# PacificBiosciences/ccs

Measured on AMD Instinct MI355X. Metric: ZMWs/sec (HiFi reads/sec), 10-pass x 10 kb synthetic, higher is better.
Workload: dtype f32

## Files before the change

ccs_amd/csrc/ccsx_kernels.hip:

```cpp
#include <hip/hip_runtime.h>
#include <stdint.h>
#include <cstdio>
#include <cstdlib>

#include "ccsx.h"
#include "ccsx_kernels.h"
#include "wave_ops.h"

#define LANDED(x) asm volatile("" : "+v"(x))

#if (defined(CCSX_EXP_NO_FILL) || defined(CCSX_EXP_NO_SCORE) || defined(CCSX_EXP_ONE_ROUND) || defined(CCSX_EXP_ALL_VALID) || defined(CCSX_EXP_CHEAP_VALIDITY) || \
     defined(CCSX_EXP_NO_ROWS) || defined(CCSX_EXP_NO_SCORE_LOG) || defined(CCSX_EXP_SKIP_ROUND2_SCORE) || defined(CCSX_EXP_NO_QV_EXP) || defined(CCSX_EXP_REPEAT) || defined(CCSX_EXP_NO_BANDMASK) || \
     defined(CCSX_EXP_HOT_PROLOGUE) || defined(CCSX_EXIT_AFTER_PROLOGUE)) && !defined(CCSX_EXPERIMENT)
#error "CCSX_EXP_* / CCSX_EXIT_AFTER_PROLOGUE switches produce wrong results: build them with -DCCSX_EXPERIMENT (never ship such a library)"
#endif
#define CCSX_STR2(x) #x
#define CCSX_STR(x) CCSX_STR2(x)
int ccsx_kernel_is_experiment()
{
#ifdef CCSX_EXPERIMENT
    return 1;
#else
    return 0;
#endif
// ... 1676 lines not shown
                    er = (kq >= 2) ? OMR[(size_t)kq * 64 + (er - loR[kq])].x : 0;
                    ent[nneed - kq] = I - er;
                }
                for (int kq = k1 + 1; kq < k2; ++kq) ent[kq] = -(1 << 20) - 64 * kq;
                dm[0] = 0u;
                for (int kq = 1; kq < nneed; ++kq) dm[kq] = 0x7fffffffu;
                P.avalid[r] = 1; P.ascore[r] = wF + wR;
            }
            continue;
        }
        if (lane == 0) {
            int32_t *ent = P.ent + P.ent_off[r];
            uint32_t *dm = P.dmask + P.ent_off[r];
            const int2 *OMF = (const int2 *)OsF, *OMR = (const int2 *)OsR;
            int e = ks ? ebF[ks] : 0;
            ent[ks] = e;
            for (int k2 = ks; k2 >= 2; --k2) { e = OMF[(size_t)k2 * 64 + (e - loF[k2])].x; ent[k2 - 1] = e; }
            ent[0] = 0;
            const int ksr = nneed - 1 - ks;
            int er = ksr ? ebR[ksr] : 0;
            for (int kq = ksr; kq >= 1; --kq) {
                er = (kq >= 2) ? OMR[(size_t)kq * 64 + (er - loR[kq])].x : 0;
                ent[nneed - kq] = I - er;
            }
            dm[0] = 0u;
            for (int k2 = 1; k2 < nneed; ++k2) dm[k2] = 0x7fffffffu;
            P.avalid[r] = 1; P.ascore[r] = wbest;
        }
      }
    }
}

__global__ void k_post(KParams P, int pass)
{
    int z = blockIdx.x * blockDim.x + threadIdx.x;
    if (z >= P.n_zmw) return;
    const int zr = P.zref[z];
    if (pass && !(zr & ZREF_PASSBIT(pass))) return;
    const bool may_retry = !P.opts.no_fallback_draft && pass < 2;
    const int retry = pass == 0 ? ZREF_RETRY : ((zr & 255) | ZREF_RETRY2);
    if (P.zstat[z] != CCSX_SUCCESS) {
        P.np[z] = 0; P.out_fn[z] = 0; P.out_rn[z] = 0;
        if (may_retry && P.zstat[z] == CCSX_DRAFT_FAILURE) P.zref[z] = retry;
        return;
    }
    int r0 = P.read_off[z], nr = P.nfull[z], np = 0, rn = 0;
    const int f0 = P.flags[r0 + (zr & 255)];
    for (int r = 0; r < nr; ++r) {
        const int v = P.avalid[r0 + r];
        np += v;
        if (v && ((P.flags[r0 + r] ^ f0) & 1)) ++rn;
    }
    P.np[z] = np; P.out_fn[z] = np - rn; P.out_rn[z] = rn;
    if (2 * np <= nr) {
        if (may_retry) P.zref[z] = retry;
        else { P.zstat[z] = CCSX_TOO_MANY_UNUSABLE; P.nwin[z] = 0; }
    }
}

__global__ __launch_bounds__(1024) void k_wmap(KParams P)
{
    __shared__ int sTot[16], sCarry;
    const int tid = threadIdx.x, lane = tid & 63, wv = tid >> 6;
    if (tid == 0) sCarry = 0;
    __syncthreads();
    for (int z0 = 0; z0 < P.n_zmw; z0 += 1024) {
        const int z = z0 + tid;
        const int v = z < P.n_zmw ? P.nwin[z] : 0;
        const int incl = wave_scan_add_i32(v);
        if (lane == 63) sTot[wv] = incl;
        __syncthreads();
        int base = sCarry;
        for (int q = 0; q < wv; ++q) base += sTot[q];
        if (z < P.n_zmw) P.wstart[z] = base + incl - v;
        __syncthreads();
        if (tid == 1023) sCarry = base + incl;
        __syncthreads();
    }
    if (tid == 0) P.wstart[P.n_zmw] = sCarry;
}
__global__ __launch_bounds__(256) void k_wmap_fill(KParams P)
{
    const int z = blockIdx.x * 4 + (threadIdx.x >> 6), lane = threadIdx.x & 63;
    if (z >= P.n_zmw) return;
    const int a = P.wstart[z], nw = P.nwin[z];
    for (int w = lane; w < nw; w += LANES) P.wslot_zmw[a + w] = z;
}

#ifndef PW_THREADS
#define PW_THREADS 256
#endif
#ifndef PW_MINWAVES
#define PW_MINWAVES 4
#endif
#define PW_WAVES (PW_THREADS / 64)
#ifndef PW_CHUNK_READS
#define PW_CHUNK_READS 8
#endif
#ifndef PW_MAXREADS
#define PW_MAXREADS 32
#endif
#ifndef PW_LDS_BYTES
#define PW_LDS_BYTES 40960
#endif
#ifndef CTXS
#define CTXS 17
#endif
#define FILL16_MAXBW 24
#define TC_LO 56
#define TC_HI 38
#define TC_ROW 32
#define TC_STRAND ((CCSX_NOBS + 1) * TC_ROW)
#define DLC_S (33 + TC_LO)
#define DLC_TOTAL (TC_LO + DLC_S + 33 + TC_HI)
#define TAB_TAIL (2 * TC_HI - 48)
#define OBS_TC(o) ((o) * (TC_ROW * 8))
#define OBS_CODE(o) ((o) * (CTXS * 8))

struct LaneMut {
    int c, q, kA, kB, isdel, fin;
    int qoff;
    float dlA, dlL;
};

__device__ __forceinline__ LaneMut lane_mut(int type, int c, int x, const uint8_t *t, int J, int lf, const float *sDL)
{
    LaneMut L;
    const int tm1 = t[c > 0 ? c - 1 : 0];
    const int nidx = (type == 2) ? c : c + 1;
    const int tn = t[nidx < 31 ? nidx : 31];
    const int fin = (type == 2) ? (c == J) : (c + 1 == J);
    const int nx = fin ? 0 : tn;
    int pA = (c > 0) ? tm1 : lf;
    const int xA = (type == 1) ? nx : x;
    if (pA > 3) pA = (xA + 2) & 3;
    const int kA = pA * 4 + xA, kB = (type == 1) ? kA : xA * 4 + nx;
    const int q = (type == 2) ? c + 1 : c + 2;
    L.c = c; L.q = q > J ? J : q; L.isdel = (type == 1); L.fin = fin; L.qoff = (type == 2) ? 0 : 1;
    L.dlA = sDL[kA]; L.dlL = sDL[kB];
    L.kA = (type == 1 && fin) ? (CTXS - 1) : kA;
    L.kB = fin ? (CTXS - 1) : kB;
    return L;
}

typedef const float __attribute__((address_space(3))) *lds_cf;
typedef const char __attribute__((address_space(3))) *lds_cc;

typedef const uint8_t __attribute__((address_space(3))) *lds_cu8;
struct ScoreChain {
    float ap, bp, acc, b, bq;
    float2 pA, pB;
    lds_cf g, be;
    lds_cu8 op;
    int dg;
};

__device__ __forceinline__ float lanes_or_zero(unsigned long long m, float v)
{
    float r;
    asm("v_cndmask_b32_e64 %0, 0, %1, %2" : "=v"(r) : "v"(v), "s"(m));
    return r;
}

__device__ __forceinline__ void score_step(ScoreChain &s, const LaneMut &L, lds_cc tA, lds_cc tB, int pitch, unsigned lim)
{
    typedef const unsigned long long __attribute__((address_space(3))) *lds_cu64;
#ifndef CCSX_EXP_NO_BANDMASK
    const unsigned long long on = __builtin_amdgcn_uicmp((unsigned)s.dg, lim, 37 );
    const float gmm = lanes_or_zero(on, *s.g);
    const float bqn = lanes_or_zero(on, *s.be);
#else
    const float gmm = *s.g, bqn = *s.be;
#endif
    const int o256 = __mul24((int)*s.op, CTXS * 8);
    const unsigned long long va = *(lds_cu64)(tA + o256), vb = *(lds_cu64)(tB + o256);
    const float2 nA = make_float2(__uint_as_float((unsigned)va), __uint_as_float((unsigned)(va >> 32)));
    const float2 nB = make_float2(__uint_as_float((unsigned)vb), __uint_as_float((unsigned)(vb >> 32)));
    s.g += pitch; s.be += pitch; s.op += 1; s.dg -= 1;
    const float insA = s.pA.y, meA = s.pA.x, insB = s.pB.y;
    const float a = __builtin_fmaf(s.ap, insA, gmm);
    float b;
    if (L.isdel) b = a;
    else b = __builtin_fmaf(s.bp, insB, __builtin_fmaf(a, L.dlA, s.ap * meA));
    s.acc = __builtin_fmaf(b, __builtin_fmaf(L.dlL, s.bq, nB.x * bqn), s.acc);
    s.ap = a; s.bp = b; s.b = b; s.pA = nA; s.pB = nB; s.bq = bqn;
}

__device__ __forceinline__ int band_row0(int c, int I, int J2, float invJ2, int J, int Wr, int nrows)
{
    const int num = __mul24(2 * c, I) + J;
    int q = (int)((float)num * invJ2);
    const int r = num - __mul24(q, J2);
    q += (r >= J2 ? 1 : 0) - (r < 0 ? 1 : 0);
    int i0 = q - Wr;
    i0 = i0 < 0 ? 0 : i0;
    const int hi = I + 1 - nrows;
    return i0 > hi ? hi : i0;
}

__device__ __forceinline__ int dq_fix(float d)
{
    if (d < -DQ_CLAMP) d = -DQ_CLAMP;
    if (d > DQ_CLAMP) d = DQ_CLAMP;
    return (int)floorf(d * DQ_SCALE + 0.5f);
}

__device__ __forceinline__ float skip_perr(int g, float floor_)
{
    if (g < 0) g = 0;
    if (g > 12) g = 12;
    const float p = 8.0f * det_exp2f(-3.0f * (float)g);
    return p < floor_ ? floor_ : p;
}

__device__ __forceinline__ int tract_len(unsigned long long m, int x, int p, int nvis)
{
    const int lo = x - p < 0 ? 0 : x - p;
    const unsigned long long cand = m & ((2ull << x) - 1ull) & ~((1ull << lo) - 1ull);
    if (!cand) return 0;
    int best = 0;
#pragma unroll
    for (int which = 0; which < 2; ++which) {
        const int k = which ? 63 - __clzll((long long)cand) : __ffsll((long long)cand) - 1;
        const unsigned long long zb = ~m & ((1ull << k) - 1ull);
        const int i = zb ? 64 - __clzll((long long)zb) : 0;
        const int j = k + (__ffsll((long long)(~m >> k)) - 1);
        const int L = j - i + p, op = ((i == 0) || (j + p >= nvis)) ? 256 : 0;
        if (L > (best & 255)) best = L | op; else if (L == (best & 255)) best |= op;
    }
    return best;
}


struct FillBand { int dlo, dhi, bw, pitch, org, rowsz; };
__device__ __forceinline__ FillBand fill_band_of(int I, int J, int S)
{
    FillBand b;
    const int dIJ = I > J ? I - J : J - I;
    const int W = SCORE_BAND + FILL_MARGIN + (dIJ > 2 ? dIJ - 2 : 0);
    const int lo = (J - I < 0 ? J - I : 0) - W, hi = (J - I > 0 ? J - I : 0) + W;
    b.dlo = lo < -I ? -I : lo; b.dhi = hi > J ? J : hi;
    b.bw = b.dhi - b.dlo + 1;
    const int bwp = b.bw | 1;
    const bool diag = bwp < S;
    b.rowsz = diag ? bwp : S; b.pitch = diag ? bwp - 1 : S; b.org = diag ? -b.dlo : 0;
    return b;
}

__device__ __forceinline__ int polish_piece_windows(int total, int slot0, int grid) { const int c = total - slot0; return c < 0 ? 0 : (c > grid ? grid : c); }
__device__ __forceinline__ int xcd_contiguous(unsigned b, int count)
{
    const int per = (count + 7) >> 3;
    const int k = (int)(b >> 3), r = (int)(b & 7u) * per + k;
    return (k < per && r < count) ? r : -1;
}

template <int PWT, int PWMIN, int PWCH>
__global__ __launch_bounds__(PWT, PWMIN) void k_polish_t(KParams P, int slot0)
{
    __shared__ float2 sCTX[(CCSX_NOBS + 1) * CTXS];
    static_assert(DLC_TOTAL >= 2 * TC_LO && TAB_TAIL >= 0 && (DLC_TOTAL & 1) == 0, "sTab: guards / alignment of sTC");
    __shared__ __attribute__((aligned(16))) float sTab[DLC_TOTAL + 2 * TC_STRAND * 2 + 48 + TAB_TAIL];
    float *const sDLC = sTab;
    float2 *const sTC = (float2 *)(sTab + DLC_TOTAL);
    float *const sDL = sTab + DLC_TOTAL + 2 * TC_STRAND * 2, *const sZP = sDL + 16;
    __shared__ uint8_t sT[2][32];
    __shared__ uint8_t sTd[32];
    uint8_t (*sObs)[68] = (uint8_t (*)[68])dyn_lds;
    float *sGB = (float *)((uint8_t *)dyn_lds + P.pw_obs_bytes);
    const int GB_FLOATS = P.pw_gb_floats;
    __shared__ int sI[PW_MAXREADS], sGoff[PW_MAXREADS], sBoff[PW_MAXREADS];
    __shared__ int sBand[PW_MAXREADS];
    __shared__ unsigned sDirty[PW_MAXREADS];
    __shared__ uint8_t sStrand[PW_MAXREADS], sRend[PW_MAXREADS];
    __shared__ unsigned sZdrop[(CCSX_MAX_PASSES + 32) / 32];
    __shared__ float sBase[PW_MAXREADS], sB00[PW_MAXREADS];
    __shared__ short2 sTask[PW_MAXREADS];
    __shared__ int sDeltaI[256];
    __shared__ uint8_t sMvalid[256];
    __shared__ int sCtl[12];
    __shared__ float sZS[4];
    __shared__ float sPskip[36];
    __shared__ uint8_t sList[256];

    const int tid = threadIdx.x, lane = tid & 63, wave = rfl(tid >> 6);
    PHASE_T0();
    const int nwin_here = polish_piece_windows(P.wstart[P.n_zmw], slot0, (int)gridDim.x);
#ifdef CCSX_EXP_HOT_PROLOGUE
    const int bid_ = slot0 + xcd_contiguous(blockIdx.x, nwin_here);
    const int bid = bid_ < slot0 ? bid_ : slot0 + ((bid_ - slot0) & 4095);
#else
    const int bid = slot0 + xcd_contiguous(blockIdx.x, nwin_here);
#endif
    if (bid < slot0) return;
    const int z = P.wslot_zmw[bid];
    const int wbo = P.wb_off[z], nw = P.nwin[z], Ld = P.draft_len[z];
    const int r0 = P.read_off[z], nreads = P.nreads_used[z];
    const int64_t so = P.seq_off[z];
    const int w = bid - P.wstart[z];
    const int32_t *wb = P.wbounds + wbo;
    const uint8_t *draft = P.draft + so;
    const int wb0 = wb[w], wb1 = wb[w + 1];
    const int64_t bo_r0 = P.base_off[r0];
    const int fl0 = P.flags[r0 + (P.zref[z] & 255)] & 1;
    int ws = wb0 - CCSX_WIN_OVERHANG; if (ws < 0) ws = 0;
    int we = wb1 + CCSX_WIN_OVERHANG; if (we > Ld) we = Ld;
    const int idx_ws = (w == 0) ? 0 : 2 * w - 1, idx_we = (w == nw - 1) ? 2 * nw - 1 : 2 * (w + 1);
    const int lfv = draft[ws > 0 ? ws - 1 : 0], rfv = draft[we < Ld ? we : Ld - 1];
    const int lf = ws > 0 ? lfv : 4, rf = we < Ld ? rfv : 4;
    const int c1 = need_col(wb, nw, Ld, idx_ws + 1), c2 = (idx_ws + 2 <= idx_we) ? need_col(wb, nw, Ld, idx_ws + 2) : we;
    const int maxins = P.opts.max_insertion_size == 0 ? 30 : P.opts.max_insertion_size;
    {
        const int e0 = tid < CCSX_NOBS * 16 ? tid : 0;
        const size_t tz = (size_t)z * 192;
        const int i0 = (e0 & 15) * CCSX_NOBS + (e0 >> 4);
        const float me0 = P.tabME[tz + i0], in0 = P.tabINS[tz + i0];
        const float dl = P.tabDL[(size_t)z * 16 + (tid & 15)];
        const float zp = P.tabZ[(size_t)z * 32 + (tid & 31)];
        const int tcl = tid < we - ws ? tid : we - ws - 1;
        const uint8_t dr = draft[ws + tcl];
        if (tid < CCSX_NOBS * 16) sCTX[(e0 >> 4) * CTXS + (e0 & 15)] = make_float2(me0, in0);
        if (tid < CTXS) sCTX[CCSX_NOBS * CTXS + tid] = make_float2(0.0f, 0.0f);
        if (tid < CCSX_NOBS) sCTX[tid * CTXS + (CTXS - 1)] = make_float2(0.0f, 0.0f);
        if (tid < TAB_TAIL) sZP[32 + tid] = 0.0f;
        if (tid < 16) sDL[tid] = dl;
        if (tid < 32) sZP[tid] = zp;
        if (tid < we - ws) { sT[0][tid] = dr; sTd[tid] = dr; }
        if (tid == 0) { sCtl[0] = we - ws; sCtl[1] = wb0 - ws; sCtl[2] = wb1 - ws; }
    }
    const int ngroups = (nreads + PW_MAXREADS - 1) / PW_MAXREADS;
    auto load_meta = [&](int g0, int ng) -> int {
        int trimflag = 0;
        const int rcl = tid < ng ? tid : ng - 1;
        const int rr = r0 + g0 + rcl;
        const int64_t bo0 = P.base_off[rr], bo1 = P.base_off[rr + 1], eo = P.ent_off[rr];
        const int flr = P.flags[rr] & 1, av = P.avalid[rr];
        const int a = P.ent[eo + idx_ws], b = P.ent[eo + idx_we];
        const unsigned m1 = P.dmask[eo + idx_ws + 1];
        const unsigned m2 = (idx_ws + 2 <= idx_we) ? P.dmask[eo + idx_ws + 2] : 0u;
// ... 82 lines not shown
            const int margin = nuse - 2 * nd;
            const bool inw = lane < J0;
            const unsigned neg = (unsigned)__ballot(inw && margin < 0);
            const unsigned nearneg = neg | (neg << 1) | (neg << 2) | (neg << 3) | (neg >> 1) | (neg >> 2) | (neg >> 3);
            const bool noheur = P.opts.disable_heuristics || (P.tflag && (P.tflag[z] & 2));
            const bool ok = inw && !noheur && margin >= SKIP_MARGIN && !((nearneg >> lane) & 1u);
            const unsigned ev = (unsigned)__ballot(ok);
            if (lane == 0) sCtl[7] = (int)ev;
            if (lane < 36) sPskip[lane] = inw ? skip_perr(margin, P.perr_floor) : 0.0f;
        }
    }
    const int half = lane >> 5, hrow = lane & 31;
    PHASE(0);
#ifdef CCSX_EXIT_AFTER_PROLOGUE
    __syncthreads();
    if (tid == 0) P.wsum[(size_t)(P.wb_off[z] - z) + w] = (float)sI[0] + (float)sObs[0][0] + sPskip[0] + sCTX[5].x;
    return;
#endif
#ifdef CCSX_EXP_REPEAT
    __syncthreads();
    const int xr_t = sT[0][tid & 31], xr_c0 = sCtl[0], xr_c1 = sCtl[1], xr_c2 = sCtl[2], xr_c7 = sCtl[7];
    const float xr_p = sPskip[tid < 36 ? tid : 0];
    for (int xrep = 0; xrep < CCSX_EXP_REPEAT; ++xrep) {
    __syncthreads();
    if (tid < 32) sT[0][tid] = (uint8_t)xr_t;
    if (tid < 36) sPskip[tid] = xr_p;
    if (tid < (CCSX_MAX_PASSES + 32) / 32) sZdrop[tid] = 0u;
    if (tid == 0) { sCtl[0] = xr_c0; sCtl[1] = xr_c1; sCtl[2] = xr_c2; sCtl[7] = xr_c7; }
    __syncthreads();
#endif
    auto plan_chunks = [&](int ng, int J, int S) {
        int r = lane;
        asm volatile("" : "+v"(r));
        const int n0 = r < ng ? sI[r] : -1;
        const FillBand fb = fill_band_of(n0 >= 0 ? n0 : 0, J, S);
        const int need0 = (2 * n0 + 3) * fb.rowsz;
        const bool qd0 = n0 <= 31 && fb.bw <= FILL16_MAXBW;
        const unsigned long long lower = (1ull << r) - 1ull;
        for (int rb = 0; rb < ng;) {
            const bool cand = n0 >= 0 && r >= rb;
            const int need = cand ? need0 : 0;
            const int incl = wave_scan_add_i32(need);
            const unsigned long long bcand = __ballot(cand);
            const unsigned long long over = __ballot(cand && (incl > GB_FLOATS || (PWCH > 0 && __popcll(bcand & lower) >= PWCH)));
            const int rend_ = over ? (int)__ffsll((long long)over) - 1 : ng;
            if (r >= rb && r < rend_) {
                if (!cand) sGoff[r] = -1;
                else {
                    const int off = incl - need;
                    sGoff[r] = off + fb.org; sBoff[r] = off + (n0 + 1) * fb.rowsz + fb.org;
                    sBand[r] = fb.pitch | (fb.rowsz << 8) | (fb.bw << 16) | ((fb.dlo + 128) << 24);
                }
            }
            const bool inchunk = cand && r < rend_;
            const bool qd = inchunk && qd0, lng = inchunk && !qd0;
            const unsigned long long bl = __ballot(lng), bs = __ballot(qd);
            const int nl_ = __popcll(bl);
            if (lng) sTask[rb + __popcll(bl & lower)].x = (short)r;
            if (qd) sTask[rb + nl_ + __popcll(bs & lower)].x = (short)r;
            if (r == rb) { sRend[rb] = (uint8_t)rend_; sTask[rb].y = (short)(nl_ | (__popcll(bs) << 8)); }
            rb = rfl(rend_);
        }
    };
    int iters = 0, nonconv = 0;
    unsigned skmask = 0;
    int nvalid_last = 0, nvfull_last = 0;
    const int nfull = P.nfull[z];
    for (int it = 0; it < CCSX_MAX_ITER; ++it) {
        __syncthreads();
        const int J = rfl(sCtl[0]);
        const unsigned evb = (unsigned)rfl(sCtl[7]);
        int tl = tid;
        asm volatile("" : "+v"(tl));
        const int ll = tl & 63;
        const int c = tl & 31;
        const int tc = (int)sT[0][c];
        const float invJ2 = 1.0f / (float)(2 * J);
        const int S = (J + 2) & ~1;
        const int lfr = (rf < 4) ? 3 - rf : 4;
        const int tm1 = wave_shr1_i32(tc, 0), tp1 = wave_shl1_i32(tc, 0);
        const int rcc = 3 - __builtin_amdgcn_ds_bpermute(((J - 1 - c) & 31) << 2, tc);
        const int rm1 = wave_shr1_i32(rcc, 0);
        if (tl < J) sT[1][tl] = (uint8_t)rcc;
        const int fctx = c < J ? ctx_of(c > 0 ? tm1 : lf, tc) : CTXS - 1;
        const int rctx = c < J ? ctx_of(c > 0 ? rm1 : lfr, rcc) : CTXS - 1;
        if (wave == (PWT / 64) - 1 && resident == 0) plan_chunks(nreads < PW_MAXREADS ? nreads : PW_MAXREADS, J, S);
        if (it == 0 && wave < 2 && P.opts.min_zscore != 0.0f) {
            static_assert(CTXS == 17 && TAB_TAIL >= 1 && CCSX_JMAX < 32, "the z-score terms of a column from J on are read at sZP[CTXS - 1] and sZP[16 + CTXS - 1]");
            const int k = wave ? rctx : fctx;
            const float t0 = sZP[k], t1 = sZP[16 + k];
            const float mu = ll < J ? t0 : 0.0f, va = ll < J ? t1 : 0.0f;
            float M = 0.0f, V = 0.0f;
#pragma unroll
            for (int q = 0; q < CCSX_JMAX; ++q) {
                M = M + __int_as_float(rl(__float_as_int(mu), q));
                V = V + __int_as_float(rl(__float_as_int(va), q));
            }
            if (lane == 0) { sZS[2 * wave] = M; sZS[2 * wave + 1] = V; }
        }
        {
            const int tcv = c < J ? tc : 9;
            const int prev = c > 0 ? (c - 1 < J ? tm1 : 8) : lf, next = c + 1 < J ? tp1 : rf;
            const bool hp = (prev == tcv) || (next == tcv);
            skmask = (unsigned)__ballot(ll < J && ((evb >> c) & 1u) && !hp);
        }
        auto lane_valid = [&](int sl) -> int {
            int v;
            if (sl < 3) v = c < J;
            else if (sl == 3) v = c < J && !(c > 0 && tm1 == tc);
            else v = c <= J && !(c > 0 && tm1 == sl - 4);
            const int cc = c < J ? c : J - 1;
            if (v && ((skmask >> cc) & 1u)) v = 0;
            else if (v && ((evb >> cc) & 1u) && !(c < J && (sl == 3 || (sl >= 4 && sl - 4 == tc)))) v = 0;
            return v;
        };
        int nvm = 0;
        {
            static_assert(PWT == 256, "the set-up: eight slots of 32 columns, two per wave");
            unsigned long long mine = 0ull;
            int basew = 0;
#pragma unroll
            for (int q = 0; q < (PWT / 64); ++q) {
                const unsigned long long b = __ballot(lane_valid(2 * q + (ll >> 5)));
                const int n = __popcll(b);
                if (q < wave) basew += n;
                if (q == wave) mine = b;
                nvm += n;
            }
            const int v0 = (int)((mine >> ll) & 1ull);
            sMvalid[tl] = (uint8_t)v0; sDeltaI[tl] = 0;
            if (v0) sList[basew + __popcll(mine & ((1ull << ll) - 1ull))] = (uint8_t)tid;
        }
        {
            static_assert(PWT == 256 && TC_ROW == 32 && 2 * TC_STRAND <= 4 * PWT && DLC_TOTAL <= PWT, "the set-up: four sTC entries and one sDLC entry per thread");
            const int row0 = tl >> 5;
            const int ej = tl - TC_LO - (tl >= TC_LO + 33 ? DLC_S : 0);
            const int both = __builtin_amdgcn_ds_bpermute((ej & 31) << 2, fctx | (rctx << 8));
            float2 v[4];
#pragma unroll
            for (int k = 0; k < 4; ++k) {
                const int r = row0 + 8 * k, sd = r >= CCSX_NOBS + 1 ? 1 : 0, o = r - sd * (CCSX_NOBS + 1);
                v[k] = sCTX[r < 2 * (CCSX_NOBS + 1) ? o * CTXS + (sd ? rctx : fctx) : 0];
            }
            const bool inw = ej >= 0 && ej < J;
            const float dv = sDL[inw ? (tl >= TC_LO + 33 ? both >> 8 : both & 255) : 0];
#pragma unroll
            for (int k = 0; k < 4; ++k) if (row0 + 8 * k < 2 * (CCSX_NOBS + 1)) sTC[tl + PWT * k] = v[k];
            if (tl < DLC_TOTAL) sDLC[tl] = tl >= DLC_TOTAL - 2 ? 0.0f : (inw ? dv : 1.0f);
        }
        const int nblk = (nvm + 63) >> 6;
        PHASE(1);
        int nvalid = 0, nvfull = 0;
        int curblk = -1;
        LaneMut LF, LR;
        int myM = 0; bool mval = false;
        for (int g0 = 0; g0 < nreads; g0 += PW_MAXREADS) {
        const int ng = nreads - g0 < PW_MAXREADS ? nreads - g0 : PW_MAXREADS;
        if (g0 != resident) {
            __syncthreads();
            const int tf = load_meta(g0, ng);
            load_obs(ng, tf);
            resident = g0;
            __syncthreads();
            if (wave == (PWT / 64) - 1) plan_chunks(ng, J, S);
        }
        int rbeg = 0;
        while (rbeg < ng) {
            __syncthreads();
            const int rend = rfl((int)sRend[rbeg]), ntasks = rfl((int)sTask[rbeg].y), nlong = ntasks & 255, nshort = ntasks >> 8;
            const short2 *const cTask = sTask + rbeg;
            PHASE(2);
#ifdef CCSX_EXP_NO_FILL
            const int nquad = 0, nunit_f = 0, rpq = 4;
#else
            const int rpq = 4;
            const int nquad = (nshort + rpq - 1) / rpq, nunit_f = 2 * nquad + 2 * nlong;
#endif
            for (int fu = wave; fu < nunit_f; fu += (PWT / 64)) {
              if (fu < 2 * nquad) {
                const int quad = fu >> 1, isb = fu & 1;
                const int g4 = lane >> 4, l16 = lane & 15;
                const int qi = rpq * quad + g4;
                const bool have = g4 < rpq && qi < nshort;
                const int myr = cTask[nlong + (have ? qi : rpq * quad)].x;
                const int I = sI[myr], sd = sStrand[myr], band = sBand[myr];
                const int pitch = band & 255, rowsz = (band >> 8) & 255, bdlo = (int)((unsigned)band >> 24) - 128, bdhi = bdlo + ((band >> 16) & 255) - 1;
                const int row0 = l16, row1 = l16 + 16;
                const bool ok0 = have && row0 <= I, ok1 = have && row1 <= I;
                const int jlo0 = (row0 + bdlo > 0) ? row0 + bdlo : 0, jhi0 = (row0 + bdhi < J) ? row0 + bdhi : J;
                const int jlo1 = (row1 + bdlo > 0) ? row1 + bdlo : 0, jhi1 = (row1 + bdhi < J) ? row1 + bdhi : J;
                int Tmax = 0;
#pragma unroll
                for (int q = 0; q < 4; ++q) { const int iq = rfl(sI[rfl((int)cTask[nlong + ((q < rpq && rpq * quad + q < nshort) ? rpq * quad + q : rpq * quad)].x)]); Tmax = iq > Tmax ? iq : Tmax; }
                Tmax += J;
                const int NEVER = 1 << 20;
#define LDPR(ROWP, OFF) (*(const float2 *)((ROWP) + (OFF)))
                if (!isb) {
                    const int obA0 = OBS_TC((row0 >= 1 && ok0) ? (int)sObs[myr][row0 - 1] : 12);
                    const int obA1 = OBS_TC(ok1 ? (int)sObs[myr][row1 - 1] : 12);
                    const char *tA = (const char *)(sTC + sd * TC_STRAND) + obA0 - 8 * row0;
                    const int dtA = obA1 - obA0 - 8 * 16;
                    const float *dA = sDLC + sd * DLC_S + (TC_LO - 1 - row0);
                    const int tA0 = ok0 ? row0 + jlo0 : NEVER, tA1 = row1 + jlo1;
                    unsigned uJ = ok0 ? (unsigned)(jhi0 - jlo0) : 0u;
                    const unsigned uJ1 = (unsigned)(jhi1 - jlo1);
                    const int tsw = ok1 ? ((row0 + jhi0) & ~3) : NEVER;
                    float *gA = sGB + sGoff[myr] + row0 * pitch - row0;
                    const int dgA = 16 * (pitch - 1), dcnt = tA0 - tA1;
                    float acur = (ok0 && row0 == 0) ? 1.0f : 0.0f, mnext = 0.0f;
#define CCSX_A_INIT(K) float dl##K = dA[K]; float2 p##K = LDPR(tA, 8 * (K));
                    CCSX_A_INIT(0) CCSX_A_INIT(1) CCSX_A_INIT(2) CCSX_A_INIT(3)
#undef CCSX_A_INIT
                    int cnt = -tA0;
#define CCSX_A_STEP(K)                                                                                                     \
                    {                                                                                                      \
                        const float up = row_ror1_f32(acur);                                              \
                        const float gmm = __builtin_fmaf(acur, dl##K, mnext);                         \
                        const unsigned long long on = __builtin_amdgcn_uicmp((unsigned)(cnt + (K)), uJ, 37 );    \
                        if (__builtin_amdgcn_inverse_ballot_w64(on)) gA[(K)] = gmm;                                        \
                        acur = lanes_or_zero(on, __builtin_fmaf(up, p##K.y, gmm));    \
                        mnext = up * p##K.x;                                                                               \
                        p##K = LDPR(tA, 8 * ((K) + 4));                            \
                        dl##K = dA[(K) + 4];                                                                               \
                    }
                    for (int t = 0; t <= Tmax; t += 4, tA += 32, dA += 4, gA += 4, cnt += 4) {
                        if (t == tsw) { tA += dtA; dA -= 16; }
                        if (t - 4 == tsw) { uJ = uJ1; cnt += dcnt; gA += dgA; }
                        CCSX_A_STEP(0) CCSX_A_STEP(1) CCSX_A_STEP(2) CCSX_A_STEP(3)
                    }
#undef CCSX_A_STEP
                    if (have && l16 == 0) sBase[myr] = sGB[sGoff[myr] + I * pitch + J];
                } else {
                    const int rowF = ok1 ? row1 : row0, jloF = ok1 ? jlo1 : jlo0, jhiF = ok1 ? jhi1 : jhi0;
                    const int obB0 = OBS_TC((ok0 && row0 < I) ? (int)sObs[myr][row0] : 12);
                    const int obBF = ok1 ? OBS_TC(row1 < I ? (int)sObs[myr][row1] : 12) : obB0;
                    const char *tB = (const char *)(sTC + sd * TC_STRAND) + obBF + 8 * (J + I - rowF);
                    const int dtB = obB0 - obBF + 8 * 16;
                    const float *dB = sDLC + sd * DLC_S + (TC_LO + J + I - rowF);
                    const int tB0 = ok0 ? I - rowF + J - jhiF : NEVER, tB1 = I - row0 + J - jhi0;
                    unsigned uJ = ok0 ? (unsigned)(jhiF - jloF) : 0u;
                    const unsigned uJ1 = (unsigned)(jhi0 - jlo0);
                    const int tsw = ok1 ? ((I - row1 + J - jlo1) & ~3) : NEVER;
                    float *bE = sGB + sBoff[myr] + rowF * pitch + (J + I - rowF);
                    const int dbE = -16 * (pitch - 1), dcnt = tB0 - tB1;
                    float bcur = (ok0 && rowF == I) ? 1.0f : 0.0f, t1next = 0.0f;
#define CCSX_B_INIT(K) float dk##K = dB[-(K)]; float2 q##K = LDPR(tB, -8 * (K));
                    CCSX_B_INIT(0) CCSX_B_INIT(1) CCSX_B_INIT(2) CCSX_B_INIT(3)
#undef CCSX_B_INIT
                    int cnt = -tB0;
#define CCSX_B_STEP(K, KN)                                                                                                 \
                    {                                                                                                      \
                        const float dn = row_rol1_f32(bcur);                                             \
                        const float bv = __builtin_fmaf(dk##K, bcur, __builtin_fmaf(q##K.y, dn, t1next));    \
                        const unsigned long long on = __builtin_amdgcn_uicmp((unsigned)(cnt + (K)), uJ, 37 );    \
                        if (__builtin_amdgcn_inverse_ballot_w64(on)) bE[-(K)] = bv;                                        \
                        bcur = lanes_or_zero(on, bv);                                                                      \
                        t1next = q##KN.x * dn;                        \
                        q##K = LDPR(tB, -8 * ((K) + 4));                                                                   \
                        dk##K = dB[-(K) - 4];                                                                              \
                    }
                    for (int t = 0; t <= Tmax; t += 4, tB -= 32, dB -= 4, bE -= 4, cnt += 4) {
                        if (t == tsw) { tB += dtB; dB += 16; }
                        if (t - 4 == tsw) { uJ = uJ1; cnt += dcnt; bE += dbE; }
                        CCSX_B_STEP(0, 1) CCSX_B_STEP(1, 2) CCSX_B_STEP(2, 3) CCSX_B_STEP(3, 0)
                    }
#undef CCSX_B_STEP
                    const int org_ = pitch == S ? 0 : -bdlo;
                    if (have) for (int x = l16; x < rowsz; x += 16) sGB[sBoff[myr] - org_ + (I + 1) * rowsz + x] = 0.0f;
                    if (have && l16 == 0) sB00[myr] = sGB[sBoff[myr]];
                }
#undef LDPR
              } else {
                const int tk = (fu - 2 * nquad) >> 1, mode = 1 + ((fu - 2 * nquad) & 1);
                const int myr = rfl((int)cTask[tk].x);
                const int row = lane;
                const int I = rfl(sI[myr]);
                const int Tmax = I + J;
                const int sd = sStrand[myr];
                const float *dlcol = sDLC + sd * DLC_S + TC_LO;
                const bool rowok = row <= I;
                const int band = sBand[myr];
                const int pitch = band & 255, rowsz = (band >> 8) & 255, bdlo = (int)((unsigned)band >> 24) - 128, bdhi = bdlo + ((band >> 16) & 255) - 1;
                const int jlo = (row + bdlo > 0) ? row + bdlo : 0, jhi = (row + bdhi < J) ? row + bdhi : J;
                const int op = OBS_TC((row >= 1 && rowok) ? (int)sObs[myr][row - 1] : 12);
                const int oc = OBS_TC((row < I) ? (int)sObs[myr][row] : 12);
                const float2 *rowA = (const float2 *)((const char *)(sTC + sd * TC_STRAND) + op), *rowB = (const float2 *)((const char *)(sTC + sd * TC_STRAND) + oc);
                const int tA0 = rowok ? row + jlo : (1 << 20), tB0 = rowok ? I - row + J - jhi : (1 << 20);
                const float one0 = (row == 0) ? 1.0f : 0.0f, oneI = (row == I) ? 1.0f : 0.0f;
                float *gA = sGB + sGoff[myr] + row * pitch - row;
                float *bB = sGB + sBoff[myr] + row * pitch + (J + I - row - 1);
                float acur = one0, updiag = 0.0f, mePrev = 0.0f, dlPrev = 1.0f;
                float bcur = oneI, dndiag = 0.0f;
                const unsigned uJ = rowok ? (unsigned)(jhi - jlo) : 0u;
                const int tAc = rowok ? row : (1 << 20);
                const unsigned uJc = (unsigned)J;
                if (mode == 1) {
                    for (int t = 0; t <= Tmax; t += 2, gA += 2) {
#define CCSX_LA_STEP(T, AOFF)                                                                                         \
                        {                                                                                                  \
                            const float up = wave_shr1_f32_z(acur);   \
                            float nv = 0.0f;                                                                               \
                            if ((unsigned)((T) - tAc) <= uJc) {              \
                                const float2 pr = rowA[(T) - row];                                                         \
                                const float dlc = dlcol[(T) - row];                                                        \
                                const float gmm = __builtin_fmaf(acur, dlPrev, updiag * mePrev);                           \
                                if ((unsigned)((T) - tA0) <= uJ) { gA[(AOFF)] = gmm; nv = __builtin_fmaf(up, pr.y, gmm); }    \
                                mePrev = pr.x; dlPrev = dlc;                                                               \
                            }                                                                                              \
                            acur = nv;                                                                                     \
                            updiag = up;                                                                                   \
                        }
                        CCSX_LA_STEP(t, 0)
                        CCSX_LA_STEP(t + 1, 1)
#undef CCSX_LA_STEP
                    }
                    if (lane == 0) sBase[myr] = sGB[sGoff[myr] + I * pitch + J];
                } else {
                    for (int t = 0; t <= Tmax; t += 2, bB -= 2) {
#define CCSX_LB_STEP(T, BOFF)                                                                                         \
                        {                                                                                                  \
                            const float dn = wave_shl1_f32_z(bcur);                                                        \
                            float nv = 0.0f;                                                                               \
                            if ((unsigned)((T) - tB0) <= uJ) {        \
                                const int jb = J + I - row - (T);                       \
                                const float2 pr = rowB[jb];                                                                \
                                const float bv = __builtin_fmaf(dlcol[jb], bcur, __builtin_fmaf(pr.y, dn, pr.x * dndiag)); \
                                bB[(BOFF)] = bv;                                                                           \
                                nv = bv;                                                                                   \
                            }                                                                                              \
                            bcur = nv;                                                                                     \
                            dndiag = dn;                                                                                   \
                        }
                        CCSX_LB_STEP(t, 1)
                        CCSX_LB_STEP(t + 1, 0)
#undef CCSX_LB_STEP
                    }
                    const int org_ = pitch == S ? 0 : -bdlo;
                    if (row < rowsz) sGB[sBoff[myr] - org_ + (I + 1) * rowsz + row] = 0.0f;
                    if (lane == 0) sB00[myr] = sGB[sBoff[myr]];
                }
              }
            }
            __syncthreads();
            PHASE(3);
            int vOk = 0; float vLa = 0.0f;
            if (lane >= rbeg && lane < rend && sGoff[lane] >= 0) {
                const float aIJ = sBase[lane], b00 = sB00[lane];
                const int I = sI[lane], sd = sStrand[lane];
                if (aIJ > TINY_P && b00 > TINY_P) {
#ifdef CCSX_EXP_CHEAP_VALIDITY
                    vLa = aIJ; const float lb = b00 - (b00 - aIJ);
#else
                    vLa = det_log2f(aIJ); const float lb = det_log2f(b00);
#endif
                    float df = vLa - lb; if (df < 0.0f) df = -df;
                    vOk = !(df > AB_TOL);
                    if ((sZdrop[g0 >> 5] >> lane) & 1u) vOk = 0;
                    else if (vOk && it == 0 && P.opts.min_zscore != 0.0f) {
                        const float zd = (vLa - (float)(2 * I)) - sZS[2 * sd];
                        const float zm = P.opts.min_zscore;
                        if (zd < 0.0f && zd * zd > (zm * zm) * sZS[2 * sd + 1]) { vOk = 0; atomicOr(&sZdrop[g0 >> 5], 1u << lane); }
                    }
                }
            }
#ifdef CCSX_EXP_ALL_VALID
            vOk = (lane >= rbeg && lane < rend && sGoff[lane] >= 0) ? 1 : 0;
#endif
            int vRlist, nv_chunk;
            {
                const bool v = vOk != 0;
                const unsigned long long bv = __ballot(v), lower = (1ull << lane) - 1ull;
                nv_chunk = rfl(__popcll(bv));
                nvfull += __popcll(bv & (nfull - g0 >= 64 ? ~0ull : (nfull - g0 <= 0 ? 0ull : (1ull << (nfull - g0)) - 1ull)));
                const int dest = v ? __popcll(bv & lower) : nv_chunk + __popcll(~bv & lower);
                vRlist = __builtin_amdgcn_ds_permute(dest << 2, lane);
            }
            PHASE(7);
            {
#ifdef CCSX_EXP_SKIP_ROUND2_SCORE
                const int nv = nv_chunk, nunits = (it == 0) ? nblk * nv : 0;
#elif defined(CCSX_EXP_NO_SCORE)
                const int nv = nv_chunk, nunits = 0;
#else
                const int nv = nv_chunk, nunits = nblk * nv;
#endif
                nvalid += nv;
                int vR, vI, vSt, vG, vB, vBd; float vBase;
                {
                    vR = lane < nv ? vRlist : rl(vRlist, 0);
                    vI = sI[vR]; vSt = (int)sStrand[vR]; vG = sGoff[vR]; vB = sBoff[vR]; vBd = sBand[vR]; vBase = __shfl(vLa, vR);
                }
                const int u_end = ((wave + 1) * nunits) / (PWT / 64);
                for (int u = (wave * nunits) / (PWT / 64); u < u_end;) {
                    int blk = 0, k0 = u;
                    while (k0 >= nv) { k0 -= nv; ++blk; }
                    const bool two = (u + 1 < u_end) && (k0 + 1 < nv);
                    u += two ? 2 : 1;
                    if (blk != curblk) {
                        curblk = blk;
                        const int li = blk * 64 + lane;
                        mval = li < nvm;
                        myM = mval ? sList[li] : 0;
                        const int slot = myM >> 5, cpos = myM & 31;
                        int type, x = 0;
                        const uint8_t *t = sT[0];
                        if (slot < 3) { type = 0; x = (t[cpos < J ? cpos : 0] + 1 + slot) & 3; }
                        else if (slot == 3) type = 1;
                        else { type = 2; x = slot - 4; }
                        if (mval) {
                            LF = lane_mut(type, cpos, x, sT[0], J, lf, sDL);
                            LR = lane_mut(type, (type == 2) ? J - cpos : J - 1 - cpos, 3 - x, sT[1], J, lfr, sDL);
                        } else { LF = lane_mut(0, 0, 0, sT[0], J, lf, sDL); LR = LF; }
                    }
                    int dq;
                    if (!two) {
                        const int ra = rl(vR, k0), Ia = rl(vI, k0);
                        const LaneMut La = rl(vSt, k0) ? LR : LF;
                        const int gA_ = rl(vG, k0), bA_ = rl(vB, k0), bdA = rl(vBd, k0);
                        const int pA = bdA & 255, dloA = (int)((unsigned)bdA >> 24) - 128; const unsigned bwA = (unsigned)(bdA >> 16) & 255u;
                        const int dA = Ia > J ? Ia - J : J - Ia, WrA = SCORE_BAND + (dA > 2 ? dA - 2 : 0);
#ifdef CCSX_EXP_NO_ROWS
                        const int nrA = 0;
#else
                        const int nrA = (Ia < 2 * WrA ? Ia : 2 * WrA) + 1;
#endif
                        const int i0a = band_row0(La.c, Ia, 2 * J, invJ2, J, WrA, nrA);
                        lds_cc tAa = (lds_cc)(sCTX + La.kA), tBa = (lds_cc)(sCTX + La.kB);
                        ScoreChain ca;
                        ca.ap = ca.bp = ca.acc = ca.b = 0.0f; ca.pA = ca.pB = make_float2(0.f, 0.f);
                        ca.g = (lds_cf)(sGB + gA_ + __mul24(i0a, pA) + La.c); ca.be = (lds_cf)(sGB + bA_ + __mul24(i0a, pA) + La.q);
                        ca.dg = La.c - i0a - dloA;
                        ca.bq = *ca.be; if ((unsigned)(La.q - i0a - dloA) >= bwA) ca.bq = 0.0f;
                        ca.be += pA;
                        const unsigned limA = bwA - 1u - (unsigned)La.qoff;
                        ca.op = (lds_cu8)(&sObs[ra][0] + i0a);
                        asm volatile("" : "+v"(ca.g), "+v"(ca.be), "+v"(tAa), "+v"(tBa), "+v"(ca.op));
                        {
                            int ia = 0;
                            for (; ia + 2 <= nrA; ia += 2) { score_step(ca, La, tAa, tBa, pA, limA); score_step(ca, La, tAa, tBa, pA, limA); }
                            if (ia < nrA) score_step(ca, La, tAa, tBa, pA, limA);
                        }
                        const float res = La.fin ? ca.b : ca.acc;
#ifdef CCSX_EXP_NO_SCORE_LOG
                        dq = __float_as_int(res) >> 20;
#else
                        dq = dq_fix(det_log2f(res) - __int_as_float(rl(__float_as_int(vBase), k0)));
#endif
                    } else {
                    const int k1 = k0 + 1;
                    const int ra = rl(vR, k0), rb = rl(vR, k1);
                    const int Ia = rl(vI, k0), Ib = rl(vI, k1);
                    const LaneMut La = rl(vSt, k0) ? LR : LF;
                    const LaneMut Lb = rl(vSt, k1) ? LR : LF;
                    const int gA_ = rl(vG, k0), bA_ = rl(vB, k0), gB_ = rl(vG, k1), bB_ = rl(vB, k1), bdA = rl(vBd, k0), bdB = rl(vBd, k1);
                    const int pA = bdA & 255, dloA = (int)((unsigned)bdA >> 24) - 128; const unsigned bwA = (unsigned)(bdA >> 16) & 255u;
                    const int pB = bdB & 255, dloB = (int)((unsigned)bdB >> 24) - 128; const unsigned bwB = (unsigned)(bdB >> 16) & 255u;
                    const int dA = Ia > J ? Ia - J : J - Ia, WrA = SCORE_BAND + (dA > 2 ? dA - 2 : 0);
                    const int nrA = (Ia < 2 * WrA ? Ia : 2 * WrA) + 1;
                    const int dB = Ib > J ? Ib - J : J - Ib, WrB = SCORE_BAND + (dB > 2 ? dB - 2 : 0);
                    const int nrB = (Ib < 2 * WrB ? Ib : 2 * WrB) + 1;
                    const int i0a = band_row0(La.c, Ia, 2 * J, invJ2, J, WrA, nrA);
                    const int i0b = band_row0(Lb.c, Ib, 2 * J, invJ2, J, WrB, nrB);
                    lds_cc tAa = (lds_cc)(sCTX + La.kA), tBa = (lds_cc)(sCTX + La.kB);
                    lds_cc tAb = (lds_cc)(sCTX + Lb.kA), tBb = (lds_cc)(sCTX + Lb.kB);
                    ScoreChain ca, cb;
                    ca.ap = ca.bp = ca.acc = ca.b = 0.0f; ca.pA = ca.pB = make_float2(0.f, 0.f);
                    cb.ap = cb.bp = cb.acc = cb.b = 0.0f; cb.pA = cb.pB = make_float2(0.f, 0.f);
                    ca.g = (lds_cf)(sGB + gA_ + __mul24(i0a, pA) + La.c); ca.be = (lds_cf)(sGB + bA_ + __mul24(i0a, pA) + La.q);
                    cb.g = (lds_cf)(sGB + gB_ + __mul24(i0b, pB) + Lb.c); cb.be = (lds_cf)(sGB + bB_ + __mul24(i0b, pB) + Lb.q);
                    ca.dg = La.c - i0a - dloA; cb.dg = Lb.c - i0b - dloB;
                    ca.bq = *ca.be; if ((unsigned)(La.q - i0a - dloA) >= bwA) ca.bq = 0.0f;
                    cb.bq = *cb.be; if ((unsigned)(Lb.q - i0b - dloB) >= bwB) cb.bq = 0.0f;
                    ca.be += pA; cb.be += pB;
                    const unsigned limA = bwA - 1u - (unsigned)La.qoff, limB = bwB - 1u - (unsigned)Lb.qoff;
                    ca.op = (lds_cu8)(&sObs[ra][0] + i0a); cb.op = (lds_cu8)(&sObs[rb][0] + i0b);
                    asm volatile("" : "+v"(ca.g), "+v"(ca.be), "+v"(cb.g), "+v"(cb.be), "+v"(tAa), "+v"(tBa), "+v"(tAb), "+v"(tBb), "+v"(ca.op), "+v"(cb.op));
                    const int nmin = nrA < nrB ? nrA : nrB;
                    int i = 0;
                    for (; i + 2 <= nmin; i += 2) {
                        score_step(ca, La, tAa, tBa, pA, limA);
                        score_step(cb, Lb, tAb, tBb, pB, limB);
                        score_step(ca, La, tAa, tBa, pA, limA);
                        score_step(cb, Lb, tAb, tBb, pB, limB);
                    }
                    for (int ia = i; ia < nrA; ++ia) score_step(ca, La, tAa, tBa, pA, limA);
                    for (int ib = i; ib < nrB; ++ib) score_step(cb, Lb, tAb, tBb, pB, limB);
                    {
                        const float res = La.fin ? ca.b : ca.acc;
                        dq = dq_fix(det_log2f(res) - __int_as_float(rl(__float_as_int(vBase), k0)));
                    }
                    {
                        const float res = Lb.fin ? cb.b : cb.acc;
                        dq += dq_fix(det_log2f(res) - __int_as_float(rl(__float_as_int(vBase), k1)));
                    }
                    }
                    if (mval) atomicAdd(&sDeltaI[myM], dq);
                }
            }
            rbeg = rend;
            PHASE(4);
        }
        }
        ++iters;
        nvalid_last = nvalid; nvfull_last = nvfull;
        __syncthreads();
        float dk[4];
        int candmask = 0;
#pragma unroll
        for (int k = 0; k < 4; ++k) {
            const int m = lane + 64 * k;
            const int mvk = sMvalid[m];
            dk[k] = (float)sDeltaI[m] * (1.0f / DQ_SCALE);
            if (mvk && dk[k] > MUT_EPS) candmask |= 1 << k;
        }
        const int anyfav = __ballot(candmask != 0) != 0ull;
#ifdef CCSX_EXP_ONE_ROUND
        break;
#endif
        if (!anyfav || P.qv_only) break;
        if (it == CCSX_MAX_ITER - 1) { nonconv = 1; break; }
        if (wave == 0) {
            int Jn = J, nacc = 0;
            unsigned accpos = 0;
            int accm = 0;
            for (;;) {
                float bd = -1.0f; int bm = 1 << 20;
#pragma unroll
                for (int k = 0; k < 4; ++k) if (candmask & (1 << k)) { const int m = lane + 64 * k; const float dv = dk[k]; if (dv > bd) { bd = dv; bm = m; } }
                const float wmax = wave_max_f32(bd);
                if (!(wmax > 0.0f)) break;
                const int msel = wave_min_i32((bd == wmax) ? bm : (1 << 20));
                if (lane == (msel & 63)) candmask &= ~(1 << (msel >> 6));
                const int sl = msel >> 5, c = msel & 31;
                if (sl >= 4 && Jn >= CCSX_JMAX) continue;
                if (sl == 3 && Jn <= JMIN_DEL + 1) continue;
                if (sl >= 4) ++Jn; else if (sl == 3) --Jn;
                if (lane == c) accm = msel;
                accpos |= 1u << c;
                ++nacc;
                if (it >= MULTI_ROUNDS) break;
                int dc = (lane & 31) - c; if (dc < 0) dc = -dc;
                if (dc < MUT_SEP) candmask = 0;
            }
            {
                int Jc = J, cs = sCtl[1], ce = sCtl[2];
                unsigned ev = (unsigned)sCtl[7];
                int tb = lane < 32 ? (int)sT[0][lane] : 0;
                float ps = lane < 36 ? sPskip[lane] : 0.0f;
                while (accpos) {
                    const int c = 31 - __clz((int)accpos);
                    accpos &= ~(1u << c);
                    const int m = rl(accm, c), sl = m >> 5;
                    if (sl < 3) { if (lane == c) tb = (tb + 1 + sl) & 3; }
                    else if (sl >= 4) {
                        const int tu = __shfl_up(tb, 1);
                        const float pu = __shfl_up(ps, 1);
                        tb = lane < c ? tb : (lane == c ? sl - 4 : tu);
                        if (lane < 32) ps = lane < c ? ps : (lane == c ? 0.0f : pu);
                        ++Jc;
                        if (c < cs) { ++cs; ++ce; } else if (c < ce) ++ce;
                        const unsigned lowm = (1u << c) - 1u;
                        ev = (ev & lowm) | ((ev & ~lowm) << 1);
                    } else {
                        const int td = __shfl_down(tb, 1);
                        const float pd = __shfl_down(ps, 1);
                        if (lane >= c) tb = td;
                        if (lane >= c && lane < 31) ps = pd;
                        --Jc;
                        if (c < cs) { --cs; --ce; } else if (c < ce) --ce;
                        const unsigned lowm = (1u << c) - 1u;
                        ev = (ev & lowm) | ((ev >> 1) & ~lowm);
                    }
                    for (int q = c - SKIP_SPREAD; q <= c + SKIP_SPREAD; ++q) if (q >= 0 && q < 32) ev &= ~(1u << q);
                }
                if (lane < 32) sT[0][lane] = (uint8_t)tb;
                if (lane < 36) sPskip[lane] = ps;
                if (lane == 0) { sCtl[0] = Jc; sCtl[1] = cs; sCtl[2] = ce; sCtl[3] = nacc; sCtl[7] = (int)ev; }
            }
        }
        __syncthreads();
        if (sCtl[3] == 0) break;
    }
    PHASE(5);
    {
        const int vmine = sMvalid[tid];
        float dv = (float)sDeltaI[tid] * (1.0f / DQ_SCALE);
        if (dv > 20.0f) dv = 20.0f;
#ifndef CCSX_EXP_NO_QV_EXP
        dv = det_exp2f(dv);
#endif
        sGB[tid] = vmine ? dv : 0.0f;
    }
    __syncthreads();
    const int J = sCtl[0], cs = sCtl[1], ce = sCtl[2];
    const size_t wi = (size_t)(P.wb_off[z] - z) + w;
    unsigned long long tm1 = 0, tm2 = 0, tm3 = 0, tm4 = 0;
    const int voff = lf < 4 ? 1 : 0;
    if (wave == 0) {
        const int nvis = J + voff + (rf < 4 ? 1 : 0);
        auto vat = [&](int i) -> int { return i < voff ? lf : (i - voff < J ? (int)sT[0][i - voff < 31 ? i - voff : 31] : rf); };
        const int vx = vat(lane);
        tm1 = __ballot(lane + 1 < nvis && vx == vat(lane + 1));
        tm2 = __ballot(lane + 2 < nvis && vx == vat(lane + 2));
        tm3 = __ballot(lane + 3 < nvis && vx == vat(lane + 3));
        tm4 = __ballot(lane + 4 < nvis && vx == vat(lane + 4));
    }
    auto has_run = [](unsigned long long m, int n) -> bool { unsigned long long x = m; for (int i = 1; i < n; ++i) x &= m >> i; return x != 0; };
    const bool any_tract = has_run(tm1, 8 - 1) || has_run(tm2, 10 - 2) || has_run(tm3, 12 - 3) || has_run(tm4, 16 - 4);
    float pl = 0.0f;
    if (tid < ce - cs) {
        const int c = cs + tid;
        float p;
        if ((skmask >> c) & 1u) p = sPskip[c];
        else {
            float s = (((unsigned)sCtl[7] >> c) & 1u) ? sPskip[c] : 0.0f;
            const bool lastc = c == J - 1;
            const int ce_ = lastc ? J : c;
            float dv[12];
#pragma unroll
            for (int sl = 0; sl < 8; ++sl) dv[sl] = sGB[sl * 32 + c];
#pragma unroll
            for (int sl = 4; sl < 8; ++sl) dv[sl + 4] = sGB[sl * 32 + ce_];
#pragma unroll
            for (int q = 0; q < 12; ++q) s = s + ((q < 8 || lastc) ? dv[q] : 0.0f);
            p = __fdiv_rn(s, 1.0f + s);
        }
        if (any_tract) {
            const int x = c + voff;
            const int nvis_ = J + voff + (rf < 4 ? 1 : 0);
            const int T1 = tract_len(tm1, x, 1, nvis_), T2 = tract_len(tm2, x, 2, nvis_), T3 = tract_len(tm3, x, 3, nvis_), T4 = tract_len(tm4, x, 4, nvis_);
            const int npw = nvalid_last;
            const float closed_scale = npw > REP_NP0 ? __fdiv_rn((float)(REP_NP0 * REP_NP0), (float)(npw * npw)) : 1.0f;
            float fl = 0.0f;
#define CCSX_TRACT_FLOOR(TT, MINL) if (((TT) & 255) >= (MINL)) { float f = __fdiv_rn(REP_ERRS, (float)((TT) & 255)); if (!((TT) & 256) && npw > REP_NP0) f = f * closed_scale; fl = f > fl ? f : fl; }
            CCSX_TRACT_FLOOR(T1, 8) CCSX_TRACT_FLOOR(T2, 10) CCSX_TRACT_FLOOR(T3, 12) CCSX_TRACT_FLOOR(T4, 16)
#undef CCSX_TRACT_FLOOR
            if (p < fl) p = fl;
        }
        if (p < P.perr_floor) p = P.perr_floor;
// ... 1864 lines not shown
```

Baseline: 41440.

## Software-pipeline score chain loads and batch observation bytes into registers

Splits the per-row score step into a load phase and a compute phase. It double-buffers them with scheduling barriers so the LDS reads for the next row overlap the FMAs of the current row. It also fetches observation bytes 12 rows at a time as aligned dwords shifted in registers, instead of one byte load per row, and packs the lane mutation descriptor into a single int to save registers. The added barriers and unpack work may constrain the compiler or add ALU ops, and the bit-field packing assumes c, q, kA and kB fit in 5 bits.

After: 42430 (median of 6 runs). 1.02x the previous value.

```diff
diff --git a/ccs_amd/csrc/ccsx_kernels.hip b/ccs_amd/csrc/ccsx_kernels.hip
--- a/ccs_amd/csrc/ccsx_kernels.hip
+++ b/ccs_amd/csrc/ccsx_kernels.hip
@@ -1852,6 +1852,7 @@
     float2 pA, pB;
     lds_cf g, be;
     lds_cu8 op;
+    unsigned w0, w1, w2;
     int dg;
 };
 
@@ -1862,21 +1863,59 @@
     return r;
 }
 
-__device__ __forceinline__ void score_step(ScoreChain &s, const LaneMut &L, lds_cc tA, lds_cc tB, int pitch, unsigned lim)
+struct LanePk { int pk; float dlA, dlL; };
+__device__ __forceinline__ LanePk lane_pack(const LaneMut &L)
+{
+    LanePk k;
+    k.pk = L.c | L.q << 5 | L.kA << 10 | L.kB << 15 | L.isdel << 20 | L.fin << 21 | L.qoff << 22;
+    k.dlA = L.dlA; k.dlL = L.dlL;
+    return k;
+}
+__device__ __forceinline__ LaneMut lane_unpack(const LanePk &k)
+{
+    LaneMut L;
+    const unsigned p = (unsigned)k.pk;
+    L.c = p & 31; L.q = (p >> 5) & 31; L.kA = (p >> 10) & 31; L.kB = (p >> 15) & 31; L.isdel = (p >> 20) & 1; L.fin = (p >> 21) & 1; L.qoff = (p >> 22) & 1;
+    L.dlA = k.dlA; L.dlL = k.dlL;
+    return L;
+}
+
+#define SCORE_OBS_ROWS 12
+typedef const unsigned __attribute__((address_space(3))) *lds_cu32;
+struct RowLoads { float g, be; unsigned long long va, vb; };
+
+__device__ __forceinline__ void obs_words(ScoreChain &s, lds_cu8 op)
+{
+    const unsigned sh = (unsigned)(unsigned long long)op & 3u;
+    lds_cu32 w = (lds_cu32)(op - sh);
+    const unsigned d0 = w[0], d1 = w[1], d2 = w[2], d3 = w[3];
+    s.w0 = __builtin_amdgcn_alignbyte(d1, d0, sh);
+    s.w1 = __builtin_amdgcn_alignbyte(d2, d1, sh);
+    s.w2 = __builtin_amdgcn_alignbyte(d3, d2, sh);
+}
+
+__device__ __forceinline__ void rs_load(ScoreChain &s, RowLoads &r, lds_cc tA, lds_cc tB, int pitch)
 {
     typedef const unsigned long long __attribute__((address_space(3))) *lds_cu64;
+    r.g = *s.g; r.be = *s.be;
+    const int o256 = __mul24((int)(s.w0 & 255u), CTXS * 8);
+    r.va = *(lds_cu64)(tA + o256); r.vb = *(lds_cu64)(tB + o256);
+    s.g += pitch; s.be += pitch;
+    s.w0 = __builtin_amdgcn_alignbit(s.w1, s.w0, 8); s.w1 = __builtin_amdgcn_alignbit(s.w2, s.w1, 8); s.w2 >>= 8;
+}
+
+__device__ __forceinline__ void rs_compute(ScoreChain &s, const LaneMut &L, const RowLoads &r, unsigned lim)
+{
 #ifndef CCSX_EXP_NO_BANDMASK
     const unsigned long long on = __builtin_amdgcn_uicmp((unsigned)s.dg, lim, 37 );
-    const float gmm = lanes_or_zero(on, *s.g);
-    const float bqn = lanes_or_zero(on, *s.be);
+    const float gmm = lanes_or_zero(on, r.g);
+    const float bqn = lanes_or_zero(on, r.be);
 #else
-    const float gmm = *s.g, bqn = *s.be;
+    const float gmm = r.g, bqn = r.be;
 #endif
-    const int o256 = __mul24((int)*s.op, CTXS * 8);
-    const unsigned long long va = *(lds_cu64)(tA + o256), vb = *(lds_cu64)(tB + o256);
-    const float2 nA = make_float2(__uint_as_float((unsigned)va), __uint_as_float((unsigned)(va >> 32)));
-    const float2 nB = make_float2(__uint_as_float((unsigned)vb), __uint_as_float((unsigned)(vb >> 32)));
-    s.g += pitch; s.be += pitch; s.op += 1; s.dg -= 1;
+    const float2 nA = make_float2(__uint_as_float((unsigned)r.va), __uint_as_float((unsigned)(r.va >> 32)));
+    const float2 nB = make_float2(__uint_as_float((unsigned)r.vb), __uint_as_float((unsigned)(r.vb >> 32)));
+    s.dg -= 1;
     const float insA = s.pA.y, meA = s.pA.x, insB = s.pB.y;
     const float a = __builtin_fmaf(s.ap, insA, gmm);
     float b;
@@ -1884,7 +1923,9 @@
     else b = __builtin_fmaf(s.bp, insB, __builtin_fmaf(a, L.dlA, s.ap * meA));
     s.acc = __builtin_fmaf(b, __builtin_fmaf(L.dlL, s.bq, nB.x * bqn), s.acc);
     s.ap = a; s.bp = b; s.b = b; s.pA = nA; s.pB = nB; s.bq = bqn;
-}
+    asm volatile("" : "+v"(s.acc), "+v"(s.bp));
+}
+#define RS_FENCE() __builtin_amdgcn_sched_barrier(0)
 
 __device__ __forceinline__ int band_row0(int c, int I, int J2, float invJ2, int J, int Wr, int nrows)
 {
@@ -2273,7 +2314,7 @@
         PHASE(1);
         int nvalid = 0, nvfull = 0;
         int curblk = -1;
-        LaneMut LF, LR;
+        LanePk LF, LR;
         int myM = 0; bool mval = false;
         for (int g0 = 0; g0 < nreads; g0 += PW_MAXREADS) {
         const int ng = nreads - g0 < PW_MAXREADS ? nreads - g0 : PW_MAXREADS;
@@ -2529,14 +2570,16 @@
                         else if (slot == 3) type = 1;
                         else { type = 2; x = slot - 4; }
                         if (mval) {
-                            LF = lane_mut(type, cpos, x, sT[0], J, lf, sDL);
-                            LR = lane_mut(type, (type == 2) ? J - cpos : J - 1 - cpos, 3 - x, sT[1], J, lfr, sDL);
-                        } else { LF = lane_mut(0, 0, 0, sT[0], J, lf, sDL); LR = LF; }
+                            LF = lane_pack(lane_mut(type, cpos, x, sT[0], J, lf, sDL));
+                            LR = lane_pack(lane_mut(type, (type == 2) ? J - cpos : J - 1 - cpos, 3 - x, sT[1], J, lfr, sDL));
+                        } else { LF = lane_pack(lane_mut(0, 0, 0, sT[0], J, lf, sDL)); LR = LF; }
                     }
                     int dq;
                     if (!two) {
                         const int ra = rl(vR, k0), Ia = rl(vI, k0);
-                        const LaneMut La = rl(vSt, k0) ? LR : LF;
+                        LanePk Ka = rl(vSt, k0) ? LR : LF;
+                        asm volatile("" : "+v"(Ka.pk));
+                        const LaneMut La = lane_unpack(Ka);
                         const int gA_ = rl(vG, k0), bA_ = rl(vB, k0), bdA = rl(vBd, k0);
                         const int pA = bdA & 255, dloA = (int)((unsigned)bdA >> 24) - 128; const unsigned bwA = (unsigned)(bdA >> 16) & 255u;
                         const int dA = Ia > J ? Ia - J : J - Ia, WrA = SCORE_BAND + (dA > 2 ? dA - 2 : 0);
@@ -2556,10 +2599,23 @@
                         const unsigned limA = bwA - 1u - (unsigned)La.qoff;
                         ca.op = (lds_cu8)(&sObs[ra][0] + i0a);
                         asm volatile("" : "+v"(ca.g), "+v"(ca.be), "+v"(tAa), "+v"(tBa), "+v"(ca.op));
-                        {
+                        for (int k = 0; k < nrA; k += SCORE_OBS_ROWS) {
+                            const int na = nrA - k < SCORE_OBS_ROWS ? nrA - k : SCORE_OBS_ROWS;
+                            obs_words(ca, ca.op + k);
+                            RowLoads X, Y;
                             int ia = 0;
-                            for (; ia + 2 <= nrA; ia += 2) { score_step(ca, La, tAa, tBa, pA, limA); score_step(ca, La, tAa, tBa, pA, limA); }
-                            if (ia < nrA) score_step(ca, La, tAa, tBa, pA, limA);
+                            rs_load(ca, X, tAa, tBa, pA);
+                            for (; ia + 3 <= na; ia += 2) {
+                                rs_load(ca, Y, tAa, tBa, pA); RS_FENCE();
+                                rs_compute(ca, La, X, limA); RS_FENCE();
+                                rs_load(ca, X, tAa, tBa, pA); RS_FENCE();
+                                rs_compute(ca, La, Y, limA); RS_FENCE();
+                            }
+                            if (ia + 2 <= na) {
+                                rs_load(ca, Y, tAa, tBa, pA); RS_FENCE();
+                                rs_compute(ca, La, X, limA); RS_FENCE();
+                                rs_compute(ca, La, Y, limA);
+                            } else rs_compute(ca, La, X, limA);
                         }
                         const float res = La.fin ? ca.b : ca.acc;
 #ifdef CCSX_EXP_NO_SCORE_LOG
@@ -2571,8 +2627,9 @@
                     const int k1 = k0 + 1;
                     const int ra = rl(vR, k0), rb = rl(vR, k1);
                     const int Ia = rl(vI, k0), Ib = rl(vI, k1);
-                    const LaneMut La = rl(vSt, k0) ? LR : LF;
-                    const LaneMut Lb = rl(vSt, k1) ? LR : LF;
+                    LanePk Ka = rl(vSt, k0) ? LR : LF, Kb = rl(vSt, k1) ? LR : LF;
+                    asm volatile("" : "+v"(Ka.pk), "+v"(Kb.pk));
+                    const LaneMut La = lane_unpack(Ka), Lb = lane_unpack(Kb);
                     const int gA_ = rl(vG, k0), bA_ = rl(vB, k0), gB_ = rl(vG, k1), bB_ = rl(vB, k1), bdA = rl(vBd, k0), bdB = rl(vBd, k1);
                     const int pA = bdA & 255, dloA = (int)((unsigned)bdA >> 24) - 128; const unsigned bwA = (unsigned)(bdA >> 16) & 255u;
                     const int pB = bdB & 255, dloB = (int)((unsigned)bdB >> 24) - 128; const unsigned bwB = (unsigned)(bdB >> 16) & 255u;
@@ -2596,16 +2653,44 @@
                     const unsigned limA = bwA - 1u - (unsigned)La.qoff, limB = bwB - 1u - (unsigned)Lb.qoff;
                     ca.op = (lds_cu8)(&sObs[ra][0] + i0a); cb.op = (lds_cu8)(&sObs[rb][0] + i0b);
                     asm volatile("" : "+v"(ca.g), "+v"(ca.be), "+v"(cb.g), "+v"(cb.be), "+v"(tAa), "+v"(tBa), "+v"(tAb), "+v"(tBb), "+v"(ca.op), "+v"(cb.op));
-                    const int nmin = nrA < nrB ? nrA : nrB;
-                    int i = 0;
-                    for (; i + 2 <= nmin; i += 2) {
-                        score_step(ca, La, tAa, tBa, pA, limA);
-                        score_step(cb, Lb, tAb, tBb, pB, limB);
-                        score_step(ca, La, tAa, tBa, pA, limA);
-                        score_step(cb, Lb, tAb, tBb, pB, limB);
+                    const int nmax = nrA > nrB ? nrA : nrB;
+                    for (int k = 0; k < nmax; k += SCORE_OBS_ROWS) {
+                        int na = nrA - k, nb = nrB - k;
+                        na = na < 0 ? 0 : (na < SCORE_OBS_ROWS ? na : SCORE_OBS_ROWS); nb = nb < 0 ? 0 : (nb < SCORE_OBS_ROWS ? nb : SCORE_OBS_ROWS);
+                        if (na > 0) obs_words(ca, ca.op + k);
+                        if (nb > 0) obs_words(cb, cb.op + k);
+                        const int nmin = na < nb ? na : nb;
+                        RowLoads X, Y;
+                        bool xl = false, yl = false;
+                        int i = 0;
+                        if (nmin >= 2) {
+                            rs_load(ca, X, tAa, tBa, pA);
+                            for (; i + 4 <= nmin; i += 2) {
+                                rs_load(cb, Y, tAb, tBb, pB); RS_FENCE();
+                                rs_compute(ca, La, X, limA); RS_FENCE();
+                                rs_load(ca, X, tAa, tBa, pA); RS_FENCE();
+                                rs_compute(cb, Lb, Y, limB); RS_FENCE();
+                                rs_load(cb, Y, tAb, tBb, pB); RS_FENCE();
+                                rs_compute(ca, La, X, limA); RS_FENCE();
+                                rs_load(ca, X, tAa, tBa, pA); RS_FENCE();
+                                rs_compute(cb, Lb, Y, limB); RS_FENCE();
+                            }
+                            rs_load(cb, Y, tAb, tBb, pB); RS_FENCE();
+                            rs_compute(ca, La, X, limA); RS_FENCE();
+                            rs_load(ca, X, tAa, tBa, pA); RS_FENCE();
+                            rs_compute(cb, Lb, Y, limB); RS_FENCE();
+                            rs_load(cb, Y, tAb, tBb, pB); RS_FENCE();
+                            rs_compute(ca, La, X, limA); RS_FENCE();
+                            i += 2;
+                            xl = i < na;
+                            if (xl) rs_load(ca, X, tAa, tBa, pA);
+                            RS_FENCE();
+                            rs_compute(cb, Lb, Y, limB); RS_FENCE();
+                        }
+                        if (i < nb) { rs_load(cb, Y, tAb, tBb, pB); yl = true; }
+                        for (int ia = i; ia < na; ++ia) { if (!xl) rs_load(ca, X, tAa, tBa, pA); xl = false; rs_compute(ca, La, X, limA); }
+                        for (int ib = i; ib < nb; ++ib) { if (!yl) rs_load(cb, Y, tAb, tBb, pB); yl = false; rs_compute(cb, Lb, Y, limB); }
                     }
-                    for (int ia = i; ia < nrA; ++ia) score_step(ca, La, tAa, tBa, pA, limA);
-                    for (int ib = i; ib < nrB; ++ib) score_step(cb, Lb, tAb, tBb, pB, limB);
                     {
                         const float res = La.fin ? ca.b : ca.acc;
                         dq = dq_fix(det_log2f(res) - __int_as_float(rl(__float_as_int(vBase), k0)));
```
